# chunhualiao/Smith-Waterman

Hardware: AMD Instinct MI355X
Metric: GCUPS (DP cell updates/s) on NxN random DNA pair (higher is better)
Workload: dtype int32; 1 GPU; 16384x16384 random DNA pair (reference generator, seed 1+rank), linear gap 3/-3/-2, int32 H + int32 P written to HBM, arg-max tracked; per_gpu=one pair per GPU, max_pos=268369846, max_score=11583, grid=256, column_tiles=1, strips=131, placement_held_gib=0, preheat_fills=640

## Files before the change

smith-waterman_amd/csrc/sw_debug.h:

```cpp
#pragma once

namespace swk {

enum DebugFlag : int {
    DBG_NO_STORES = 1 << 0,
    DBG_PRODUCER_ONLY = 1 << 1,
    DBG_GENERIC_PRODUCER = 1 << 2,
    DBG_SKIP_STRIP1 = 1 << 3,
    DBG_NO_PERM = 1 << 4,
    DBG_NO_POLL_BACKOFF = 1 << 5,
    DBG_WAVE_PLACEMENT = 1 << 6,
    DBG_BLOCK_STAMPS = 1 << 7,
    DBG_NO_CONSUMER_LOOP = 1 << 8,
    DBG_EDGE_DUMP = 1 << 9,
    DBG_EPOCH8_WRAP_EARLY = 1 << 10,
    DBG_POISON_HALO = 1 << 11,
    DBG_ONE_IMPORTER = 1 << 12,
    DBG_PROGRESS_FORM = 1 << 13,
    DBG_NO_TWO_COLUMNS = 1 << 14,
    DBG_FORCE_TWO_COLUMNS = 1 << 15,
    DBG_BATCH_SINGLE_PAIR = 1 << 16,
    DBG_NO_SCOUTS = 1 << 17,
    DBG_BATCH_NO_WAVE16 = 1 << 18,
    DBG_NO_TILES = 1 << 19,
    DBG_NO_SPLIT = 1 << 20,
    DBG_BATCH_NO_PACKED_P = 1 << 21,
    DBG_S2_SCOUTS_NO_EXPORT = 1 << 21,
    DBG_S2_SYNTH_HALO = 1 << 22,
    DBG_NO_XCD_DEALING = 1 << 23,
    DBG_S2_IMPORTERS = 3 << 24,
    DBG_NO_PACING = 1 << 27,
    DBG_S2_BARRIER_SCAN = 1 << 28,
    DBG_S2_SCAN_ALL = 1 << 29,
};
constexpr int DBG_S2_IMPORTERS_SHIFT = 24;
constexpr int DBG_BATCH_MASK = DBG_NO_STORES | DBG_PRODUCER_ONLY | DBG_GENERIC_PRODUCER;

}
```

smith-waterman_amd/csrc/sw_systolic2.inc:

```

constexpr int S2_W = 126;
template <bool OV> __device__ __forceinline__ constexpr int s2_stride() { return OV ? 110 : S2_W; }
template <bool OV> __device__ __forceinline__ constexpr int s2_xlane() { return s2_stride<OV>() >> 1; }

struct S2Side {
    __attribute__((aligned(16))) u32 halo[SY_RH];
    __attribute__((aligned(16))) u32 lowv[128];
    int topv[128];
    int prod_u, halo_ready, never, pad;
};
struct Sys2Lds {
    __attribute__((aligned(16))) unsigned char ringA[64 * SY_LSTR];
    __attribute__((aligned(16))) unsigned char ringB[64 * SY_LSTR];
    __attribute__((aligned(16))) int cons_blk[8];
    S2Side side;
};

#define P2_STEP(GA, GB, GA1, GB1, TAP, TAN, TBP, TBN, HIN, SA, SB, BYTE)                                                   \
    "v_add_u32 v121, v121, %[ngap]\n\t"                                                                                   \
    "v_max3_i32 v120, " TBP ", " GB1 ", v121\n\t"                                                                         \
    "v_max3_i32 v122, " TAP ", " GB1 ", v121\n\t"                                                                         \
    "v_add_u32_sdwa " TBN ", " GB1 ", sext(" SA ") dst_sel:DWORD dst_unused:UNUSED_PAD src0_sel:DWORD src1_sel:" BYTE "\n\t" \
    "v_max_i32_dpp " GA ", v120, " GA1 " wave_shr:1 row_mask:0xf bank_mask:0xf\n\t"                                       \
    "v_max3_i32 " GB ", v122, " GA ", " HIN "\n\t"                                                                        \
// ... 109 lines not shown
    "s_cbranch_scc1 LgoB" #KB "_%=\n\t"                                                                                   \
    "s_add_i32 s89, s89, 1\n\t"                                                                                           \
    "s_add_i32 s95, s95, 1\n\t"                                                                                           \
    "s_cmp_lt_u32 s89, 0x1000000\n\t"                                                                                     \
    "s_cbranch_scc1 LpollB" #KB "_%=\n\t"                                                                                 \
    "s_branch Lfail_%=\n"

#define C2_P32(PA, PB, PP, POL) "buffer_store_dwordx2 " PP ", %[voffP], %[rP], s82 offen" POL "\n\t"
#define C2_P8(PA, PB, PP, POL)                                                                                             \
    "buffer_store_byte " PA ", %[voffP], %[rP], s82 offen" POL "\n\t"                                                      \
    "buffer_store_byte " PB ", %[voffP], %[rP], s82 offen offset:1" POL "\n\t"
#define C2_NOTRK(HA, HB, K2) ""
#define C2_TRK(HA, HB, K2)                                                                                                 \
    "v_cmp_gt_i32_e64 s[72:73], " HA ", %[bv]\n\t"                                                                         \
    "v_max_i32 %[bv], %[bv], " HA "\n\t"                                                                                   \
    "v_cndmask_b32_e64 %[bi], %[bi], " K2 ", s[72:73]\n\t"                                                                 \
    "v_cmp_gt_i32_e64 s[72:73], " HB ", %[bv]\n\t"                                                                         \
    "v_max_i32 %[bv], %[bv], " HB "\n\t"                                                                                   \
    "v_cndmask_b32_e64 %[bi], %[bi], " K2 "+1, s[72:73]\n\t"
#define C2_ROW(GA0, GA1, GB0, GB1, CH, BYTE, HA, HB, HP, PA, PB, PP, POL, HST, PST, TRK, K2)                                    \
    "v_sub_u32 %[nz], %[nz], %[ngap]\n\t"                                                                                 \
    "v_cmp_eq_u32_sdwa s[68:69], %[aA], " CH " src0_sel:DWORD src1_sel:" BYTE "\n\t"                                       \
    "v_cmp_eq_u32_sdwa s[70:71], %[aB], " CH " src0_sel:DWORD src1_sel:" BYTE "\n\t"                                       \
    "v_add_u32 " HA ", " GA1 ", %[nz]\n\t"                                                                                \
    "v_add3_u32 " HB ", " GB1 ", %[nz], v112\n\t"                                                                     \
    "v_cndmask_b32_e64 v113, %[xm], %[mm], s[68:69]\n\t"                                                                  \
    "v_cndmask_b32_e64 v114, %[xm], %[mm], s[70:71]\n\t"                                                                  \
    HST(HP, POL)                                                                                                           \
    "v_cmp_eq_u32_e64 s[60:61], " GA0 ", " GA1 "\n\t"                                                                     \
    "v_cmp_eq_u32_e64 s[64:65], " GB0 ", " GB1 "\n\t"                                                                     \
    "v_add_u32_dpp v115, " GB0 ", v113 wave_shr:1 row_mask:0xf bank_mask:0xf bound_ctrl:0\n\t"                            \
    "v_add_u32 v116, " GA0 ", v114\n\t"                                                                                   \
    "v_cndmask_b32_e64 " PA ", 2, 1, s[60:61]\n\t"                                                                        \
    "v_cndmask_b32_e64 " PB ", 2, 1, s[64:65]\n\t"                                                                        \
    "v_cmp_eq_u32_e64 s[62:63], v115, " GA1 "\n\t"                                                                        \
    "v_cmp_eq_u32_e64 s[66:67], v116, " GB1 "\n\t"                                                                        \
    "v_max3_i32 %[bm], %[bm], " HA ", " HB "\n\t"                                                                         \
    "v_cmp_eq_u32_e64 s[68:69], 0, " HA "\n\t"                                                                            \
    "v_cndmask_b32_e64 " PA ", " PA ", 3, s[62:63]\n\t"                                                                   \
    "v_cndmask_b32_e64 " PB ", " PB ", 3, s[66:67]\n\t"                                                                   \
    "v_cmp_eq_u32_e64 s[70:71], 0, " HB "\n\t"                                                                            \
    "s_add_u32 s80, s80, %[rowbH]\n\t"                                                                                    \
    "v_cndmask_b32_e64 " PA ", " PA ", 0, s[68:69]\n\t"                                                                   \
    TRK(HA, HB, K2)                                                                                                        \
    "v_cndmask_b32_e64 " PB ", " PB ", 0, s[70:71]\n\t"                                                                   \
    PST(PA, PB, PP, POL)                                                                                                   \
    "s_add_u32 s82, s82, %[rowbP]\n\t"
#define C2_H32(HP, POL) "buffer_store_dwordx2 " HP ", %[voffH], %[rH], s80 offen" POL "\n\t"
#define C2_H64(HP, POL) "buffer_store_dwordx4 " HP ", %[voffH], %[rH], s80 offen" POL "\n\t"
#define C2_EV32(GA0, GA1, GB0, GB1, CH, BYTE, POL, PST, TRK, K2) C2_ROW(GA0, GA1, GB0, GB1, CH, BYTE, "v100", "v101", "v[100:101]", "v102", "v103", "v[102:103]", POL, C2_H32, PST, TRK, K2)
#define C2_OD32(GA0, GA1, GB0, GB1, CH, BYTE, POL, PST, TRK, K2) C2_ROW(GA0, GA1, GB0, GB1, CH, BYTE, "v104", "v105", "v[104:105]", "v106", "v107", "v[106:107]", POL, C2_H32, PST, TRK, K2)
#define C2_EV64(GA0, GA1, GB0, GB1, CH, BYTE, POL, PST, TRK, K2) C2_ROW(GA0, GA1, GB0, GB1, CH, BYTE, "v100", "v102", "v[100:103]", "v104", "v105", "v[104:105]", POL, C2_H64, PST, TRK, K2)
#define C2_OD64(GA0, GA1, GB0, GB1, CH, BYTE, POL, PST, TRK, K2) C2_ROW(GA0, GA1, GB0, GB1, CH, BYTE, "v106", "v108", "v[106:109]", "v110", "v111", "v[110:111]", POL, C2_H64, PST, TRK, K2)
#define C2_RD(K, KB, OFF) "ds_read_b32 v" #K ", %[ea] offset:" #OFF "\n\tds_read_b32 v" #KB ", %[eb] offset:" #OFF "\n\t"
#define C2_RDW(K, KB, I)                                                                                                   \
    "v_add_u32 v98, " #I ", %[ew]\n\t"                                                                                   \
    "v_and_b32 v98, 1020, v98\n\t"                                                                                        \
    "v_add_u32 v99, v98, %[eb]\n\t"                                                                                       \
    "v_add_u32 v98, v98, %[ea]\n\t"                                                                                       \
    "ds_read_b32 v" #K ", v98\n\t"                                                                                        \
    "ds_read_b32 v" #KB ", v99\n\t"
#define C2_READS_FLAT                                                                                                      \
    C2_RD(64, 81, 0) C2_RD(65, 82, 4) C2_RD(66, 83, 8) C2_RD(67, 84, 12) C2_RD(68, 85, 16) C2_RD(69, 86, 20) C2_RD(70, 87, 24) C2_RD(71, 88, 28)      \
    C2_RD(72, 89, 32) C2_RD(73, 90, 36) C2_RD(74, 91, 40) C2_RD(75, 92, 44) C2_RD(76, 93, 48) C2_RD(77, 94, 52) C2_RD(78, 95, 56) C2_RD(79, 96, 60) \
    C2_RD(80, 97, 64)
#define C2_READS_WRAP                                                                                                      \
    C2_RDW(64, 81, 0) C2_RDW(65, 82, 4) C2_RDW(66, 83, 8) C2_RDW(67, 84, 12) C2_RDW(68, 85, 16) C2_RDW(69, 86, 20) C2_RDW(70, 87, 24)              \
    C2_RDW(71, 88, 28) C2_RDW(72, 89, 32) C2_RDW(73, 90, 36) C2_RDW(74, 91, 40) C2_RDW(75, 92, 44) C2_RDW(76, 93, 48) C2_RDW(77, 94, 52)            \
    C2_RDW(78, 95, 56) C2_RDW(79, 96, 60) C2_RDW(80, 97, 64)
#define C2_ASM(READS, POL, PST, TRK, C2_EV, C2_OD)                                                                                       \
    asm volatile(                                                                                                          \
        "s_load_dwordx4 s[76:79], %[cptr], 0x0\n\t"                                                                       \
        READS                                                                                                              \
        "ds_write_b32 %[slot], %[qv]\n\t"            \
        "s_mov_b32 s80, 0\n\t"                                                                                            \
        "s_mov_b32 s82, 0\n\t"                                                                                            \
        "v_sub_u32 v112, 0, %[ngap]\n\t"                                                                                  \
        "v_mov_b32 v101, 0\n\tv_mov_b32 v103, 0\n\tv_mov_b32 v107, 0\n\tv_mov_b32 v109, 0\n\t"    \
        "s_waitcnt lgkmcnt(0)\n\t"                                    \
        "s_cmp_lg_u32 %[first], 0\n\t"                                                                                    \
        "s_cbranch_scc0 Lc2_%=\n\t"                                                                                       \
        "v_mov_b32 v64, %[g0a]\n\t"                  \
        "v_mov_b32 v81, %[g0b]\n"                                                                                          \
        "Lc2_%=:\n\t"                                                                                                     \
        C2_EV("v64", "v65", "v81", "v82", "s76", "BYTE_0", POL, PST, TRK, "0") C2_OD("v65", "v66", "v82", "v83", "s76", "BYTE_1", POL, PST, TRK, "2")       \
        C2_EV("v66", "v67", "v83", "v84", "s76", "BYTE_2", POL, PST, TRK, "4") C2_OD("v67", "v68", "v84", "v85", "s76", "BYTE_3", POL, PST, TRK, "6")       \
        C2_EV("v68", "v69", "v85", "v86", "s77", "BYTE_0", POL, PST, TRK, "8") C2_OD("v69", "v70", "v86", "v87", "s77", "BYTE_1", POL, PST, TRK, "10")      \
        C2_EV("v70", "v71", "v87", "v88", "s77", "BYTE_2", POL, PST, TRK, "12") C2_OD("v71", "v72", "v88", "v89", "s77", "BYTE_3", POL, PST, TRK, "14")     \
        C2_EV("v72", "v73", "v89", "v90", "s78", "BYTE_0", POL, PST, TRK, "16") C2_OD("v73", "v74", "v90", "v91", "s78", "BYTE_1", POL, PST, TRK, "18")     \
        C2_EV("v74", "v75", "v91", "v92", "s78", "BYTE_2", POL, PST, TRK, "20") C2_OD("v75", "v76", "v92", "v93", "s78", "BYTE_3", POL, PST, TRK, "22")     \
        C2_EV("v76", "v77", "v93", "v94", "s79", "BYTE_0", POL, PST, TRK, "24") C2_OD("v77", "v78", "v94", "v95", "s79", "BYTE_1", POL, PST, TRK, "26")     \
        C2_EV("v78", "v79", "v95", "v96", "s79", "BYTE_2", POL, PST, TRK, "28") C2_OD("v79", "v80", "v96", "v97", "s79", "BYTE_3", POL, PST, TRK, "30")     \
        "v_mov_b32 %[gla], v80\n\t"                      \
        "v_mov_b32 %[glb], v97\n\t"                                                                                       \
        : [nz] "+v"(nz), [bm] "+v"(bm), [bv] "+v"(bv), [bi] "+v"(bi), [gla] "=&v"(gla), [glb] "=&v"(glb)                    \
        : [ea] "v"(ea), [eb] "v"(eb), [ew] "v"(ew), [slot] "v"(slot_addr), [qv] "v"(qv), [first] "s"(first), [g0a] "v"(g0a), [g0b] "v"(g0b),  \
          [aA] "v"(aA), [aB] "v"(aB), [mm] "v"(mm_v), [xm] "v"(xm_v), [ngap] "v"(ngap_v), [voffH] "v"(voffH),           \
          [voffP] "v"(voffP), [rH] "s"(rH), [rP] "s"(rP), [rowbH] "s"(rowbH), [rowbP] "s"(rowbP), [cptr] "s"(chars)           \
        : "vcc", "scc", "memory", "s60", "s61", "s62", "s63", "s64", "s65", "s66", "s67", "s68", "s69", "s70", "s71", "s72", "s73", "s76", "s77", "s78", "s79", \
          "s80", "s82", "v64", "v65", "v66", "v67", "v68", "v69", "v70", "v71", "v72", "v73", "v74", "v75", "v76", "v77", "v78", "v79", "v80", "v81", "v82",    \
          "v83", "v84", "v85", "v86", "v87", "v88", "v89", "v90", "v91", "v92", "v93", "v94", "v95", "v96", "v97", "v98", "v99", "v100", "v101", "v102", \
          "v103", "v104", "v105", "v106", "v107", "v108", "v109", "v110", "v111", "v112", "v113", "v114", "v115", "v116")
struct C2Out { u32 bm, gla, glb; };
__device__ __forceinline__ C2Out consumer_block2(bool flat, bool nt, bool p8, bool trk, bool h64, u32 ea, u32 eb, u32 ew, u32 slot_addr, u32 qv, int first, u32 g0a,
                                                 u32 g0b, u32& nz, u32& bv, u32& bi, u32 aA, u32 aB, u32 mm_v, u32 xm_v, u32 ngap_v, u32 voffH,
                                                 u32 voffP, sw_i32x4 rH, sw_i32x4 rP, u32 rowbH, u32 rowbP, const unsigned char* chars) {
    u32 bm = 0, gla, glb;
#define C2_PICK(READS)                                                                                                     \
    if (h64) {                                                           \
        if (p8) { if (nt) { C2_ASM(READS, " nt", C2_P8, C2_NOTRK, C2_EV64, C2_OD64); } else { C2_ASM(READS, "", C2_P8, C2_NOTRK, C2_EV64, C2_OD64); } }        \
        else { if (nt) { C2_ASM(READS, " nt", C2_P32, C2_NOTRK, C2_EV64, C2_OD64); } else { C2_ASM(READS, "", C2_P32, C2_NOTRK, C2_EV64, C2_OD64); } }         \
    } else if (trk) {                                                                                                      \
        if (p8) { if (nt) { C2_ASM(READS, " nt", C2_P8, C2_TRK, C2_EV32, C2_OD32); } else { C2_ASM(READS, "", C2_P8, C2_TRK, C2_EV32, C2_OD32); } }            \
        else { if (nt) { C2_ASM(READS, " nt", C2_P32, C2_TRK, C2_EV32, C2_OD32); } else { C2_ASM(READS, "", C2_P32, C2_TRK, C2_EV32, C2_OD32); } }             \
    } else {                                                                                                               \
        if (p8) { if (nt) { C2_ASM(READS, " nt", C2_P8, C2_NOTRK, C2_EV32, C2_OD32); } else { C2_ASM(READS, "", C2_P8, C2_NOTRK, C2_EV32, C2_OD32); } }        \
        else { if (nt) { C2_ASM(READS, " nt", C2_P32, C2_NOTRK, C2_EV32, C2_OD32); } else { C2_ASM(READS, "", C2_P32, C2_NOTRK, C2_EV32, C2_OD32); } }         \
    }
    if (flat) { C2_PICK(C2_READS_FLAT) } else { C2_PICK(C2_READS_WRAP) }
#undef C2_PICK
    return C2Out{bm, gla, glb};
}

#include "sw_wholeline_consumer.inc"

#include "sw_filler_producer.inc"


#define P2S_TAIL(GB0, GB3, H0, H3, WO, HADDR)                                                                              \
    "buffer_store_dwordx4 v[" GB0 ":" GB3 "], v97, s[76:79], s75 offen offset:" WO P2S_EXP_MOD "\n\t"                       \
    "ds_read_b128 v[" H0 ":" H3 "], " HADDR "\n\t"
#define P2S_LGKM "3"
#ifndef P2S_VMCNT
// ... 58 lines not shown
                const uint64_t now = __builtin_amdgcn_s_memrealtime();
                if (t0 == 0) t0 = now;
                if (((now - t0) >> 10) > (uint64_t)p.top_wait_ticks)
                    __hip_atomic_store((gu32*)p.abort_flag, 1u, __ATOMIC_RELAXED, __HIP_MEMORY_SCOPE_AGENT);
                if (__builtin_amdgcn_readfirstlane((int)__hip_atomic_load((gu32*)p.abort_flag, __ATOMIC_RELAXED, __HIP_MEMORY_SCOPE_AGENT)) != 0) break;
            }
        }
        tv = (int)(u32)gr;
    } else if (p.top && want) {
        tv = p.top[jt];
    }
    sd.topv[tid] = tv;
}

struct S2Pace {
    bool on = false, set = false;
    int S = 0, s = 0, steps = 0, bps = 0;
    float inv = 0.f, start = 0.f;
    __device__ __forceinline__ void calibrate(const FillParams& p, float t_first) {
        int tau_ps = p.filler_tau_ps, hop_ps = p.filler_hop_ps, bw_gbs = p.filler_bw_gbs;
        asm volatile("" : "+s"(tau_ps), "+s"(hop_ps), "+s"(bw_gbs));
        const float tau_min = (float)tau_ps * 1e-4f, hop_host = (float)hop_ps * 1e-4f;
        const float bw_per_tick = (float)bw_gbs * 10.f, fsteps = (float)steps;
        const float hop = (s >= 8) ? fminf(fmaxf(t_first / (float)s, 0.5f * hop_host), 1.5f * hop_host) : hop_host;
        start = (s >= 8) ? t_first : (float)s * hop;
        const float esteps = p.filler_end_steps > 0 ? (float)p.filler_end_steps : fsteps;
        const float wsteps = p.filler_full_steps > 0 ? (float)p.filler_full_steps : fsteps;
        const float d_chain = (float)(S - 1) * hop + esteps * tau_min;
        const float x = bw_per_tick * hop / ((float)max(bps, 1) * wsteps);
        const float d_bw = (x < 20.f) ? (float)S * hop / (1.f - __expf(-x)) : 0.f;
        const float d = fmaxf(d_chain, d_bw);
        inv = (d > start + 1.f) ? fsteps / (d - start) : 0.f;
        set = true;
    }
};
template <bool OV>
__device__ __forceinline__ bool s2_importer(S2Side& sd, const FillParams& p, int s_real, int phi, int UT, int rows, int gb, int ngap, int lane, bool synth = false,
                                            S2Pace pace = S2Pace(), int stop_u = 0x7fffffff) {
    const int s = synth ? 0 : s_real;
    __builtin_amdgcn_s_setprio(2);
    const u32 row0v = (u32)(gb + sd.topv[0] + ngap * s_real * s2_stride<OV>());
    const int xl = s2_xlane<OV>();
    const int ulast = min(UT + 64, stop_u);
    const u32 tag = (u32)gb >> 24;
    const u32* e4 = (s > 0) ? p.edge4 + (int64_t)(s - 1) * p.e4stride : nullptr;
    int impu = 1;
    bool wide = true;
    Spin spin; spin.code = 3;
    const uint64_t pace_t0 = __builtin_amdgcn_s_memrealtime();
    while (impu <= ulast) {
        const int front = lds_load(&sd.halo_ready);
        if (front > 1) impu = max(impu, front);
        if (impu > ulast) break;
        int lim = min(ulast + 1, lds_load(&sd.prod_u) + SY_RH / 2 - 2 * SY_U);
        if (pace.set && pace.inv > 0.f) lim = min(lim, 64 + max(0, (int)(((float)(uint32_t)(__builtin_amdgcn_s_memrealtime() - pace_t0) - pace.start) * pace.inv)));
        int base = impu;
        auto windows = [&](auto NB) {
            constexpr int nbat = decltype(NB)::value;
            u32 vals[nbat];
            bool oks[nbat];
#pragma unroll
            for (int b4 = 0; b4 < nbat; ++b4) {
                const int u = impu + b4 * 64 + lane;
                const int r = u - phi;
                u32 v = row0v;
                bool ok = true;
                if (r > rows) v = (u32)gb;
                else if (r > 0) {
                    if (s == 0) v = (u32)(gb + ngap * r + (p.tile_left ? p.tile_left[(int64_t)r * p.M] : 0));
                    else {
                        v = __hip_atomic_load((gu32*)(e4 + u + xl), __ATOMIC_RELAXED, __HIP_MEMORY_SCOPE_AGENT);
                        ok = (v >> 24) == tag;
                    }
                }
                vals[b4] = v;
                oks[b4] = ok && (u < lim);
            }
            const int front2 = lds_load(&sd.halo_ready);
#pragma unroll
            for (int b4 = 0; b4 < nbat; ++b4) {
                const int u = impu + b4 * 64 + lane;
                const u64 okm = __ballot(oks[b4]);
                const int npre = (okm == ~0ull) ? 64 : __builtin_ctzll(~okm);
                if (base == impu + b4 * 64 && npre > 0) {
                    if (lane < npre && (front2 <= 1 || u >= front2)) {
                        __hip_atomic_store(&sd.halo[(u - 1) & (SY_RH - 1)], vals[b4], __ATOMIC_RELAXED, __HIP_MEMORY_SCOPE_WORKGROUP);
                        __hip_atomic_store(&sd.halo[(u - 1 + SY_RH / 2) & (SY_RH - 1)], 0u, __ATOMIC_RELAXED, __HIP_MEMORY_SCOPE_WORKGROUP);
                    }
                    base += npre;
                }
            }
        };
        if (wide) windows(std::integral_constant<int, 4>{});
        else windows(std::integral_constant<int, 1>{});
        wide = (base - impu) >= 64;
        if (base > impu) {
            asm volatile("" ::: "memory");
            if (pace.on && !pace.set && base > phi + 1)
                pace.calibrate(p, (float)(uint32_t)(__builtin_amdgcn_s_memrealtime() - pace_t0));
            impu = base;
            __hip_atomic_fetch_max(&sd.halo_ready, impu, __ATOMIC_RELAXED, __HIP_MEMORY_SCOPE_WORKGROUP);
        } else if (spin.fail(p.abort_flag)) {
            return false;
        }
    }
    __builtin_amdgcn_s_setprio(0);
    return true;
}
// ... 471 lines not shown
                const bool nostore = (p.debug_flags & DBG_NO_STORES) != 0;
                const bool nt = p.store_nt != 0, store_h = H != nullptr && !nostore, store_p = P != nullptr && !nostore, trk = H == nullptr;
                const u32 voffH = (okB && store_h) ? (u32)jA * (h64 ? 8u : 4u) : SY_OOB, voffP = (okB && store_p) ? (u32)jA * (p8 ? 1u : 4u) : SY_OOB;
                const u32 rowbH = (u32)(M * (h64 ? 8 : 4)), rowbP = (u32)(M * (p8 ? 1 : 4));
                int bestcode = 0;
                constexpr int W = s2_stride<OV>();
                const bool allod = (M & 1) == 0;
                const bool wlaunch = OV && H != nullptr && !(P != nullptr && p8 && (h64 || allod)) && !trk && !p.bot_gran && !has_top &&
                                     ((uintptr_t)H & (h64 ? 15u : 7u)) == 0 && ((uintptr_t)P & 7u) == 0;
                const bool wl = wlaunch && s > 0 && s < S - 1;
                const bool mine = !OV || wlaunch || s == S - 1 || lane <= (W >> 1);
                u32 wm = 0;
                if (wl) {
                    const int64_t c1 = (int64_t)s * W + 1;
                    const u32 f0H = (u32)(((uint64_t)(uintptr_t)H + (uint64_t)(((M + c1) * 4) << hsh)) & 63u), f0P = (u32)(((uint64_t)(uintptr_t)P + (uint64_t)((M + c1) * 4)) & 63u);
                    const u32 pszH = h64 ? 16u : 8u, spanH = h64 ? 880u : 440u;
#pragma nounroll
                    for (int k = 0; k < SY_U; ++k) {
                        const bool odr = allod || (k & 1);
                        const u32 pcH = pszH * (u32)(lane - 1) - (odr ? pszH / 2 : 0u), pcP = 8u * (u32)(lane - 1) - (odr ? 4u : 0u);
                        if (!((u32)(pcH - ((f0H + (u32)k * rowbH + pcH) & 63u)) < spanH)) wm |= 1u << k;
                        if (!((u32)(pcP - ((f0P + (u32)k * rowbP + pcP) & 63u)) < 440u)) wm |= 1u << (16 + k);
                    }
                }
                if (has_top && store_h && k9 == 0) {
                    if (h64) {
                        if (okA) ((int64_t*)H)[jA] = topA;
                        if (okB) ((int64_t*)H)[jB] = topB;
                        if (s == 0 && lane == 0) ((int64_t*)H)[0] = topB;
                    } else {
                        if (okA) H[jA] = topA;
                        if (okB) H[jB] = topB;
                        if (s == 0 && lane == 0) H[0] = topB;
                    }
                }
                for (int q = q_lo + k9; q < nblk; q += nc_eff) {
                    const int qs = __builtin_amdgcn_readfirstlane(q);
                    const int r0 = qs * SY_U + 1;
                    const int need = r0 + SY_U - 1 + 63 + phi;
                    if (sf && q == q_lo + k9 && need > 256) {
                        if (!s2_importer<OV>(sd, p, s, phi, UT, rows, gb, ngap, lane, false, S2Pace(), need - 192)) return;
                    }
                    while (lds_load(&sd.prod_u) < need)
                        if (spin.fail(p.abort_flag)) return;
                    asm volatile("" ::: "memory");
                    const u32 e0 = (u32)(r0 - 2 + lane + phi);
                    const bool flat = (((u32)(r0 - 2 + phi) & (SY_R - 1)) + 63 + SY_U) < (u32)SY_R;
                    const uint64_t bH = (uint64_t)(uintptr_t)(H + (((int64_t)r0 * M) << hsh)), bP = (uint64_t)(uintptr_t)(P + (int64_t)r0 * M * (p8 ? 1 : 4));
                    const int nbr = min(SY_U, rows - r0 + 1);
                    const int nrH = nbr == SY_U ? 0x7FFFFF00 : nbr * (int)rowbH, nrP = nbr == SY_U ? 0x7FFFFF00 : nbr * (int)rowbP;
                    const sw_i32x4 dH = {__builtin_amdgcn_readfirstlane((int)(u32)bH), __builtin_amdgcn_readfirstlane((int)(u32)(bH >> 32)), nrH, 0x00020000};
                    const sw_i32x4 dP = {__builtin_amdgcn_readfirstlane((int)(u32)bP), __builtin_amdgcn_readfirstlane((int)(u32)(bP >> 32)), nrP, 0x00020000};
                    u32 nz = (u32)(-(gb + ngap * (r0 - 1 + (int)jA)));
                    u32 bv = (u32)best, bi = 0;
                    const u32 eoff = (e0 & (SY_R - 1)) * 4u;
                    C2Out o;
                    if (wl) {
                        const int64_t c1 = (int64_t)s * W + 1;
                        const uint64_t fH = bH + (uint64_t)((c1 * 4) << hsh), fP = bP + (uint64_t)(c1 * 4);
                        const uint64_t bH2 = fH & ~(uint64_t)63, bP2 = fP & ~(uint64_t)63;
                        const u32 dlH = (u32)(bH2 - bH), dlP = (u32)(bP2 - bP);
                        const sw_i32x4 dH2 = {__builtin_amdgcn_readfirstlane((int)(u32)bH2), __builtin_amdgcn_readfirstlane((int)(u32)(bH2 >> 32)),
                                              nbr == SY_U ? 0x7FFFFF00 : __builtin_amdgcn_readfirstlane(nrH - (int)dlH), 0x00020000};
                        const sw_i32x4 dP2 = {__builtin_amdgcn_readfirstlane((int)(u32)bP2), __builtin_amdgcn_readfirstlane((int)(u32)(bP2 >> 32)),
                                              nbr == SY_U ? 0x7FFFFF00 : __builtin_amdgcn_readfirstlane(nrP - (int)dlP), 0x00020000};
                        const u32 vH = voffH == SY_OOB ? SY_OOB : voffH - dlH;
                        const u32 vP = p8 ? ((voffP == SY_OOB || lane > (W >> 1)) ? SY_OOB : voffP) : (voffP == SY_OOB ? SY_OOB : voffP - dlP);
                        o.bm = consumer_block3(flat, nt, h64, p8, flat ? laneA + eoff : laneA, flat ? laneB + eoff : laneB, eoff, slot_addr, (u32)qs,
                                               __builtin_amdgcn_readfirstlane(qs == 0 ? 1 : 0), g0a, g0b, nz, (u32)aA, (u32)aB, mm_v, xm_v, ngap_v, vH, vP,
                                               dH2, p8 ? dP : dP2, rowbH, rowbP, bchars + (r0 - 1), wm, allod);
                        o.gla = o.glb = 0u;
                    } else
                    o = consumer_block2(flat, nt, p8, trk, h64, flat ? laneA + eoff : laneA, flat ? laneB + eoff : laneB, eoff, slot_addr, (u32)qs,
                                                    __builtin_amdgcn_readfirstlane(qs == 0 ? 1 : 0), g0a, g0b, nz, bv, bi, (u32)aA, (u32)aB, mm_v, xm_v, ngap_v,
                                                    voffH, voffP, dH, dP, rowbH, rowbP, bchars + (r0 - 1));
                    if (trk) { if (okB && mine && (int)bv > best) { best = (int)bv; bestq = qs; bestcode = (int)bi; } }
                    else if (okB && mine && (int)o.bm > best) { best = (int)o.bm; bestq = qs; }
                    if (p.bot_gran && qs == nblk - 1) {
                        const int zl = gb + ngap * (rows + (int)jA);
                        if (okA) __hip_atomic_store((gu64*)(p.bot_gran + jA), ((u64)p.bot_tag << 32) | (u64)(u32)((int)o.gla - zl), __ATOMIC_RELAXED, __HIP_MEMORY_SCOPE_SYSTEM);
                        if (okB) __hip_atomic_store((gu64*)(p.bot_gran + jB), ((u64)p.bot_tag << 32) | (u64)(u32)((int)o.glb - zl - ngap), __ATOMIC_RELAXED, __HIP_MEMORY_SCOPE_SYSTEM);
                        if (s == 0 && lane == 0) __hip_atomic_store((gu64*)p.bot_gran, (u64)p.bot_tag << 32, __ATOMIC_RELAXED, __HIP_MEMORY_SCOPE_SYSTEM);
                        if (p.bot_done) {
                            __builtin_amdgcn_fence(__ATOMIC_RELEASE, "");
                            asm volatile("s_waitcnt vmcnt(0)" ::: "memory");
                            const int n63 = (int)((p.cols + 62) / 63);
                            if (lane < 2 && 2 * s + lane < n63)
                                __hip_atomic_store((gu32*)(p.bot_done + 2 * s + lane), p.bot_tag, __ATOMIC_RELAXED, __HIP_MEMORY_SCOPE_SYSTEM);
                        }
                    }
                }
                if (best > 0 && !nostore) {
                    if (trk) {
                        bestrow = bestq * SY_U + 1 + (bestcode >> 1);
                        bestcol = bestcode & 1;
                    } else {
                        __builtin_amdgcn_s_waitcnt(0);
                        const u32 psz = h64 ? 16u : 8u, span = h64 ? 880u : 440u, lc = psz * (u32)(lane - 1);
                        const u32 f0 = (u32)(((uint64_t)(uintptr_t)H + (uint64_t)(((((int64_t)bestq * SY_U + 1) * M + (int64_t)s * W + 1) * 4) << hsh)) & 63u);
                        auto inwin = [&](u32 rowoff, u32 pc) { return (u32)(pc - ((f0 + rowoff + pc) & 63u)) < span; };
                        const int nk = min(SY_U, rows - bestq * SY_U);
                        int hvA[SY_U], hvB[SY_U];
#pragma unroll
                        for (int k = 0; k < SY_U; ++k) {
                            const int64_t o = (int64_t)(bestq * SY_U + 1 + min(k, nk - 1)) * M + jA;
                            hvA[k] = (int)__builtin_nontemporal_load(&H[o << hsh]);
                            hvB[k] = (int)__builtin_nontemporal_load(&H[(o + 1) << hsh]);
                        }
#pragma unroll
                        for (int k = SY_U - 1; k >= 0; --k) {
                            bool stA = k < nk, stB = k < nk;
                            if (wl) {
                                const u32 rowoff = (u32)k * rowbH;
                                if (allod || (k & 1)) { stA = stA && inwin(rowoff, lc - psz / 2); stB = stB && lane < 63 && inwin(rowoff, lc + psz / 2); }
                                else stA = stB = stA && inwin(rowoff, lc);
                            }
                            if (stB && hvB[k] == best) { bestrow = bestq * SY_U + 1 + k; bestcol = 1; }
                            if (stA && hvA[k] == best) { bestrow = bestq * SY_U + 1 + k; bestcol = 0; }
                        }
                        if (bestrow == 0 && wlaunch) best = 0;
                    }
                }
            } else
            for (int q = q_lo + k9; q < nblk; q += nc_eff) {
                const int r0 = q * SY_U + 1;
                const int need = r0 + SY_U - 1 + 63 + phi;
                while (lds_load(&sd.prod_u) < need)
// ... 106 lines not shown
```

smith-waterman_amd/csrc/sw_wholeline_consumer.inc:

```

#define C3_MASK(BIT, VOFF)                                                                                                 \
    "v_bfe_i32 v124, %[wm], " BIT ", 1\n\t"                                                                                \
    "v_or_b32 v120, v124, " VOFF "\n\t"
#define C3_ROW(GA0, GA1, GB0, GB1, CH, BYTE, HA, HB, PA, PB, HST, PST)                                                     \
    "v_sub_u32 %[nz], %[nz], %[ngap]\n\t"                                                                                 \
    "v_cmp_eq_u32_sdwa s[68:69], %[aA], " CH " src0_sel:DWORD src1_sel:" BYTE "\n\t"                                       \
    "v_cmp_eq_u32_sdwa s[70:71], %[aB], " CH " src0_sel:DWORD src1_sel:" BYTE "\n\t"                                       \
    "v_add_u32 " HA ", " GA1 ", %[nz]\n\t"                                                                                \
    "v_add3_u32 " HB ", " GB1 ", %[nz], v112\n\t"                                                                         \
    "v_cndmask_b32_e64 v113, %[xm], %[mm], s[68:69]\n\t"                                                                  \
    "v_cndmask_b32_e64 v114, %[xm], %[mm], s[70:71]\n\t"                                                                  \
    HST                                                                                                                    \
    "v_cmp_eq_u32_e64 s[60:61], " GA0 ", " GA1 "\n\t"                                                                     \
    "v_cmp_eq_u32_e64 s[64:65], " GB0 ", " GB1 "\n\t"                                                                     \
    "v_add_u32_dpp v115, " GB0 ", v113 wave_shr:1 row_mask:0xf bank_mask:0xf bound_ctrl:0\n\t"                            \
    "v_add_u32 v99, " GA0 ", v114\n\t"                                                                                   \
    "v_cndmask_b32_e64 " PA ", 2, 1, s[60:61]\n\t"                                                                        \
    "v_cndmask_b32_e64 " PB ", 2, 1, s[64:65]\n\t"                                                                        \
    "v_cmp_eq_u32_e64 s[62:63], v115, " GA1 "\n\t"                                                                        \
    "v_cmp_eq_u32_e64 s[66:67], v99, " GB1 "\n\t"                                                                        \
    "v_max3_i32 %[bm], %[bm], " HA ", " HB "\n\t"                                                                         \
    "v_cmp_eq_u32_e64 s[68:69], 0, " HA "\n\t"                                                                            \
    "v_cndmask_b32_e64 " PA ", " PA ", 3, s[62:63]\n\t"                                                                   \
    "v_cndmask_b32_e64 " PB ", " PB ", 3, s[66:67]\n\t"                                                                   \
    "v_cmp_eq_u32_e64 s[70:71], 0, " HB "\n\t"                                                                            \
    "s_add_u32 s80, s80, %[rowbH]\n\t"                                                                                    \
    "v_cndmask_b32_e64 " PA ", " PA ", 0, s[68:69]\n\t"                                                                   \
    "v_cndmask_b32_e64 " PB ", " PB ", 0, s[70:71]\n\t"                                                                   \
    PST                                                                                                                    \
    "s_add_u32 s82, s82, %[rowbP]\n\t"
#define C3_EV32(GA0, GA1, GB0, GB1, CH, BYTE, POL, KH, KP)                                                                         \
    C3_ROW(GA0, GA1, GB0, GB1, CH, BYTE, "v100", "v101", "v102", "v103",                                                   \
           C3_MASK(KH, "%[voffH]") "buffer_store_dwordx2 v[100:101], v120, %[rH], s80 offen" POL "\n\t",  \
           C3_MASK(KP, "%[voffP]") "buffer_store_dwordx2 v[102:103], v120, %[rP], s82 offen" POL "\n\t")
#define C3_EV32P8(GA0, GA1, GB0, GB1, CH, BYTE, POL, KH, KP)                                                                       \
    C3_ROW(GA0, GA1, GB0, GB1, CH, BYTE, "v100", "v101", "v102", "v103",                                                   \
           C3_MASK(KH, "%[voffH]") "buffer_store_dwordx2 v[100:101], v120, %[rH], s80 offen" POL "\n\t",                    \
           "buffer_store_byte v102, %[voffP], %[rP], s82 offen\n\tbuffer_store_byte v103, %[voffP], %[rP], s82 offen offset:1\n\t")
#define C3_OD32P8(GA0, GA1, GB0, GB1, CH, BYTE, POL, KH, KP)                                                                       \
    C3_ROW(GA0, GA1, GB0, GB1, CH, BYTE, "v119", "v121", "v123", "v125",                                                   \
           "v_mov_b32_dpp v118, v121 wave_shr:1 row_mask:0xf bank_mask:0xf bound_ctrl:0\n\t"                              \
           C3_MASK(KH, "v116") "buffer_store_dwordx2 v[118:119], v120, %[rH], s80 offen" POL "\n\t",                        \
           "buffer_store_byte v123, %[voffP], %[rP], s82 offen\n\tbuffer_store_byte v125, %[voffP], %[rP], s82 offen offset:1\n\t")
#define C3_EV64(GA0, GA1, GB0, GB1, CH, BYTE, POL, KH, KP)                                                                         \
    C3_ROW(GA0, GA1, GB0, GB1, CH, BYTE, "v100", "v102", "v104", "v105",                                                   \
           C3_MASK(KH, "%[voffH]") "buffer_store_dwordx4 v[100:103], v120, %[rH], s80 offen" POL "\n\t",  \
           C3_MASK(KP, "%[voffP]") "buffer_store_dwordx2 v[104:105], v120, %[rP], s82 offen" POL "\n\t")
#define C3_OD_P(POL, KP)                                                                                                       \
           C3_MASK(KP, "v117")    \
           "v_mov_b32_dpp v122, v125 wave_shr:1 row_mask:0xf bank_mask:0xf bound_ctrl:0\n\t"                              \
           "buffer_store_dwordx2 v[122:123], v120, %[rP], s82 offen" POL "\n\t"
#define C3_OD32(GA0, GA1, GB0, GB1, CH, BYTE, POL, KH, KP)                                                                         \
    C3_ROW(GA0, GA1, GB0, GB1, CH, BYTE, "v119", "v121", "v123", "v125",                                                   \
           "v_mov_b32_dpp v118, v121 wave_shr:1 row_mask:0xf bank_mask:0xf bound_ctrl:0\n\t"                              \
           C3_MASK(KH, "v116") "buffer_store_dwordx2 v[118:119], v120, %[rH], s80 offen" POL "\n\t", \
           C3_OD_P(POL, KP))
#define C3_OD64(GA0, GA1, GB0, GB1, CH, BYTE, POL, KH, KP)                                                                         \
    C3_ROW(GA0, GA1, GB0, GB1, CH, BYTE, "v108", "v110", "v123", "v125",                                                   \
           "v_mov_b32_dpp v106, v110 wave_shr:1 row_mask:0xf bank_mask:0xf bound_ctrl:0\n\t"                              \
           C3_MASK(KH, "v116") "buffer_store_dwordx4 v[106:109], v120, %[rH], s80 offen" POL "\n\t", \
           C3_OD_P(POL, KP))
#define C3_ASM(READS, POL, C3_EV, C3_OD, HALFH)                                                                                   \
    asm volatile(                                                                                                          \
        "s_load_dwordx4 s[76:79], %[cptr], 0x0\n\t"                                                                       \
        READS                                                                                                              \
        "ds_write_b32 %[slot], %[qv]\n\t"            \
        "s_mov_b32 s80, 0\n\t"                                                                                            \
        "s_mov_b32 s82, 0\n\t"                                                                                            \
        "v_sub_u32 v112, 0, %[ngap]\n\t"                                                                                  \
        "v_add_u32 v116, " HALFH ", %[voffH]\n\t"                  \
        "v_add_u32 v117, -4, %[voffP]\n\t"                                                                                \
        "v_mov_b32 v101, 0\n\tv_mov_b32 v103, 0\n\tv_mov_b32 v107, 0\n\tv_mov_b32 v109, 0\n\tv_mov_b32 v111, 0\n\t"    \
        "s_waitcnt lgkmcnt(0)\n\t"                                    \
        "s_cmp_lg_u32 %[first], 0\n\t"                                                                                    \
        "s_cbranch_scc0 Lc3_%=\n\t"                                                                                       \
        "v_mov_b32 v64, %[g0a]\n\t"                  \
        "v_mov_b32 v81, %[g0b]\n"                                                                                          \
        "Lc3_%=:\n\t"                                                                                                     \
        C3_EV("v64", "v65", "v81", "v82", "s76", "BYTE_0", POL, "0", "16") C3_OD("v65", "v66", "v82", "v83", "s76", "BYTE_1", POL, "1", "17")     \
        C3_EV("v66", "v67", "v83", "v84", "s76", "BYTE_2", POL, "2", "18") C3_OD("v67", "v68", "v84", "v85", "s76", "BYTE_3", POL, "3", "19")     \
        C3_EV("v68", "v69", "v85", "v86", "s77", "BYTE_0", POL, "4", "20") C3_OD("v69", "v70", "v86", "v87", "s77", "BYTE_1", POL, "5", "21")     \
        C3_EV("v70", "v71", "v87", "v88", "s77", "BYTE_2", POL, "6", "22") C3_OD("v71", "v72", "v88", "v89", "s77", "BYTE_3", POL, "7", "23")     \
        C3_EV("v72", "v73", "v89", "v90", "s78", "BYTE_0", POL, "8", "24") C3_OD("v73", "v74", "v90", "v91", "s78", "BYTE_1", POL, "9", "25")     \
        C3_EV("v74", "v75", "v91", "v92", "s78", "BYTE_2", POL, "10", "26") C3_OD("v75", "v76", "v92", "v93", "s78", "BYTE_3", POL, "11", "27")     \
        C3_EV("v76", "v77", "v93", "v94", "s79", "BYTE_0", POL, "12", "28") C3_OD("v77", "v78", "v94", "v95", "s79", "BYTE_1", POL, "13", "29")     \
        C3_EV("v78", "v79", "v95", "v96", "s79", "BYTE_2", POL, "14", "30") C3_OD("v79", "v80", "v96", "v97", "s79", "BYTE_3", POL, "15", "31")     \
        : [nz] "+v"(nz), [bm] "+v"(bm)                                                                                      \
        : [ea] "v"(ea), [eb] "v"(eb), [ew] "v"(ew), [slot] "v"(slot_addr), [qv] "v"(qv), [first] "s"(first), [g0a] "v"(g0a), [g0b] "v"(g0b),  \
          [aA] "v"(aA), [aB] "v"(aB), [mm] "v"(mm_v), [xm] "v"(xm_v), [ngap] "v"(ngap_v), [voffH] "v"(voffH),           \
          [voffP] "v"(voffP), [wm] "v"(wm), [rH] "s"(rH), [rP] "s"(rP), [rowbH] "s"(rowbH), [rowbP] "s"(rowbP), [cptr] "s"(chars)     \
        : "vcc", "scc", "memory", "s60", "s61", "s62", "s63", "s64", "s65", "s66", "s67", "s68", "s69", "s70", "s71", "s72", "s73", "s76", "s77", "s78", "s79", \
          "s80", "s82",                                \
          "v64", "v65", "v66", "v67", "v68", "v69", "v70", "v71", "v72", "v73", "v74", "v75", "v76", "v77", "v78", "v79", "v80", "v81", "v82",    \
          "v83", "v84", "v85", "v86", "v87", "v88", "v89", "v90", "v91", "v92", "v93", "v94", "v95", "v96", "v97", "v98", "v99", "v100", "v101", "v102", \
          "v103", "v104", "v105", "v106", "v107", "v108", "v109", "v110", "v111", "v112", "v113", "v114", "v115", "v116", "v117", "v118", "v119", "v120", \
          "v121", "v122", "v123", "v124", "v125", "v126", "v127")
__device__ __forceinline__ u32 consumer_block3(bool flat, bool nt, bool h64, bool p8, u32 ea, u32 eb, u32 ew, u32 slot_addr, u32 qv, int first, u32 g0a, u32 g0b, u32& nz,
                                               u32 aA, u32 aB, u32 mm_v, u32 xm_v, u32 ngap_v, u32 voffH, u32 voffP, sw_i32x4 rH, sw_i32x4 rP,
                                               u32 rowbH, u32 rowbP, const unsigned char* chars, u32 wm, bool allod) {
    u32 bm = 0;
#define C3_PICK(READS)                                                                                                     \
    if (p8) {                                                                       \
        if (nt) { C3_ASM(READS, " nt", C3_EV32P8, C3_OD32P8, "-4"); } else { C3_ASM(READS, "", C3_EV32P8, C3_OD32P8, "-4"); }           \
    } else if (allod) {                                                                                                    \
        if (h64) { if (nt) { C3_ASM(READS, " nt", C3_OD64, C3_OD64, "-8"); } else { C3_ASM(READS, "", C3_OD64, C3_OD64, "-8"); } }    \
        else { if (nt) { C3_ASM(READS, " nt", C3_OD32, C3_OD32, "-4"); } else { C3_ASM(READS, "", C3_OD32, C3_OD32, "-4"); } }        \
    } else if (h64) { if (nt) { C3_ASM(READS, " nt", C3_EV64, C3_OD64, "-8"); } else { C3_ASM(READS, "", C3_EV64, C3_OD64, "-8"); } } \
    else { if (nt) { C3_ASM(READS, " nt", C3_EV32, C3_OD32, "-4"); } else { C3_ASM(READS, "", C3_EV32, C3_OD32, "-4"); } }
    if (flat) { C3_PICK(C2_READS_FLAT) } else { C3_PICK(C2_READS_WRAP) }
#undef C3_PICK
    return bm;
}
```

Baseline: 337.9 GCUPS.

## Pair LDS ring reads with ds_read2 and sleep importers when blocked

Replaces the 34 single ds_read_b32 loads in the flat consumer ring read with paired ds_read2_b32 instructions, halving the LDS instruction count. Importer waves that cannot advance, because they are blocked by the ring limit or by pacing, now drop priority and s_sleep for a duration scaled to the pacing rate instead of spinning, which frees issue slots for compute waves. A debug bit that skips ring reads is also added, routed through the first flag. The sleeps may add latency when the producer advances sooner than expected.

```diff
diff --git a/smith-waterman_amd/csrc/sw_debug.h b/smith-waterman_amd/csrc/sw_debug.h
--- a/smith-waterman_amd/csrc/sw_debug.h
+++ b/smith-waterman_amd/csrc/sw_debug.h
@@ -29,9 +29,11 @@
     DBG_S2_SYNTH_HALO = 1 << 22,
     DBG_NO_XCD_DEALING = 1 << 23,
     DBG_S2_IMPORTERS = 3 << 24,
+    DBG_S2_NO_RING_READS = 1 << 26,
     DBG_NO_PACING = 1 << 27,
     DBG_S2_BARRIER_SCAN = 1 << 28,
     DBG_S2_SCAN_ALL = 1 << 29,
+    DBG_S2_IMPORTERS_POLL = 1 << 30,
 };
 constexpr int DBG_S2_IMPORTERS_SHIFT = 24;
 constexpr int DBG_BATCH_MASK = DBG_NO_STORES | DBG_PRODUCER_ONLY | DBG_GENERIC_PRODUCER;
diff --git a/smith-waterman_amd/csrc/sw_systolic2.inc b/smith-waterman_amd/csrc/sw_systolic2.inc
--- a/smith-waterman_amd/csrc/sw_systolic2.inc
+++ b/smith-waterman_amd/csrc/sw_systolic2.inc
@@ -185,7 +185,7 @@
 #define C2_OD32(GA0, GA1, GB0, GB1, CH, BYTE, POL, PST, TRK, K2) C2_ROW(GA0, GA1, GB0, GB1, CH, BYTE, "v104", "v105", "v[104:105]", "v106", "v107", "v[106:107]", POL, C2_H32, PST, TRK, K2)
 #define C2_EV64(GA0, GA1, GB0, GB1, CH, BYTE, POL, PST, TRK, K2) C2_ROW(GA0, GA1, GB0, GB1, CH, BYTE, "v100", "v102", "v[100:103]", "v104", "v105", "v[104:105]", POL, C2_H64, PST, TRK, K2)
 #define C2_OD64(GA0, GA1, GB0, GB1, CH, BYTE, POL, PST, TRK, K2) C2_ROW(GA0, GA1, GB0, GB1, CH, BYTE, "v106", "v108", "v[106:109]", "v110", "v111", "v[110:111]", POL, C2_H64, PST, TRK, K2)
-#define C2_RD(K, KB, OFF) "ds_read_b32 v" #K ", %[ea] offset:" #OFF "\n\tds_read_b32 v" #KB ", %[eb] offset:" #OFF "\n\t"
+#define C2_RD2(K0, K1, ADDR, O0, O1) "ds_read2_b32 v[" #K0 ":" #K1 "], %[" #ADDR "] offset0:" #O0 " offset1:" #O1 "\n\t"
 #define C2_RDW(K, KB, I)                                                                                                   \
     "v_add_u32 v98, " #I ", %[ew]\n\t"                                                                                   \
     "v_and_b32 v98, 1020, v98\n\t"                                                                                        \
@@ -194,9 +194,12 @@
     "ds_read_b32 v" #K ", v98\n\t"                                                                                        \
     "ds_read_b32 v" #KB ", v99\n\t"
 #define C2_READS_FLAT                                                                                                      \
-    C2_RD(64, 81, 0) C2_RD(65, 82, 4) C2_RD(66, 83, 8) C2_RD(67, 84, 12) C2_RD(68, 85, 16) C2_RD(69, 86, 20) C2_RD(70, 87, 24) C2_RD(71, 88, 28)      \
-    C2_RD(72, 89, 32) C2_RD(73, 90, 36) C2_RD(74, 91, 40) C2_RD(75, 92, 44) C2_RD(76, 93, 48) C2_RD(77, 94, 52) C2_RD(78, 95, 56) C2_RD(79, 96, 60) \
-    C2_RD(80, 97, 64)
+    "ds_read_b32 v81, %[eb]\n\t"                                                                                         \
+    C2_RD2(64, 65, ea, 0, 1) C2_RD2(82, 83, eb, 1, 2) C2_RD2(66, 67, ea, 2, 3) C2_RD2(84, 85, eb, 3, 4)                    \
+    C2_RD2(68, 69, ea, 4, 5) C2_RD2(86, 87, eb, 5, 6) C2_RD2(70, 71, ea, 6, 7) C2_RD2(88, 89, eb, 7, 8)                    \
+    C2_RD2(72, 73, ea, 8, 9) C2_RD2(90, 91, eb, 9, 10) C2_RD2(74, 75, ea, 10, 11) C2_RD2(92, 93, eb, 11, 12)               \
+    C2_RD2(76, 77, ea, 12, 13) C2_RD2(94, 95, eb, 13, 14) C2_RD2(78, 79, ea, 14, 15) C2_RD2(96, 97, eb, 15, 16)            \
+    "ds_read_b32 v80, %[ea] offset:64\n\t"
 #define C2_READS_WRAP                                                                                                      \
     C2_RDW(64, 81, 0) C2_RDW(65, 82, 4) C2_RDW(66, 83, 8) C2_RDW(67, 84, 12) C2_RDW(68, 85, 16) C2_RDW(69, 86, 20) C2_RDW(70, 87, 24)              \
     C2_RDW(71, 88, 28) C2_RDW(72, 89, 32) C2_RDW(73, 90, 36) C2_RDW(74, 91, 40) C2_RDW(75, 92, 44) C2_RDW(76, 93, 48) C2_RDW(77, 94, 52)            \
@@ -204,14 +207,17 @@
 #define C2_ASM(READS, POL, PST, TRK, C2_EV, C2_OD)                                                                                       \
     asm volatile(                                                                                                          \
         "s_load_dwordx4 s[76:79], %[cptr], 0x0\n\t"                                                                       \
+        "s_bitcmp1_b32 %[first], 1\n\t"              \
+        "s_cbranch_scc1 Lnr_%=\n\t"                                                                                       \
         READS                                                                                                              \
+        "Lnr_%=:\n\t"                                                                                                     \
         "ds_write_b32 %[slot], %[qv]\n\t"            \
         "s_mov_b32 s80, 0\n\t"                                                                                            \
         "s_mov_b32 s82, 0\n\t"                                                                                            \
         "v_sub_u32 v112, 0, %[ngap]\n\t"                                                                                  \
         "v_mov_b32 v101, 0\n\tv_mov_b32 v103, 0\n\tv_mov_b32 v107, 0\n\tv_mov_b32 v109, 0\n\t"    \
         "s_waitcnt lgkmcnt(0)\n\t"                                    \
-        "s_cmp_lg_u32 %[first], 0\n\t"                                                                                    \
+        "s_bitcmp1_b32 %[first], 0\n\t"                                               \
         "s_cbranch_scc0 Lc2_%=\n\t"                                                                                       \
         "v_mov_b32 v64, %[g0a]\n\t"                  \
         "v_mov_b32 v81, %[g0b]\n"                                                                                          \
@@ -376,8 +382,23 @@
         const int front = lds_load(&sd.halo_ready);
         if (front > 1) impu = max(impu, front);
         if (impu > ulast) break;
-        int lim = min(ulast + 1, lds_load(&sd.prod_u) + SY_RH / 2 - 2 * SY_U);
+        const int ring_lim = lds_load(&sd.prod_u) + SY_RH / 2 - 2 * SY_U;
+        int lim = min(ulast + 1, ring_lim);
         if (pace.set && pace.inv > 0.f) lim = min(lim, 64 + max(0, (int)(((float)(uint32_t)(__builtin_amdgcn_s_memrealtime() - pace_t0) - pace.start) * pace.inv)));
+        if (impu >= lim && !(p.debug_flags & DBG_S2_IMPORTERS_POLL)) {
+            __builtin_amdgcn_s_setprio(0);
+            if (lim == ring_lim) __builtin_amdgcn_s_sleep(60);
+            else {
+                if (pace.inv <= 0.125f) __builtin_amdgcn_s_sleep(48);
+                else if (pace.inv <= 0.25f) __builtin_amdgcn_s_sleep(24);
+                else if (pace.inv <= 0.5f) __builtin_amdgcn_s_sleep(12);
+                else __builtin_amdgcn_s_sleep(6);
+            }
+            wide = false;
+            if (spin.fail(p.abort_flag)) return false;
+            __builtin_amdgcn_s_setprio(2);
+            continue;
+        }
         int base = impu;
         auto windows = [&](auto NB) {
             constexpr int nbat = decltype(NB)::value;
@@ -955,6 +976,9 @@
                     const sw_i32x4 dH = {__builtin_amdgcn_readfirstlane((int)(u32)bH), __builtin_amdgcn_readfirstlane((int)(u32)(bH >> 32)), nrH, 0x00020000};
                     const sw_i32x4 dP = {__builtin_amdgcn_readfirstlane((int)(u32)bP), __builtin_amdgcn_readfirstlane((int)(u32)(bP >> 32)), nrP, 0x00020000};
                     u32 nz = (u32)(-(gb + ngap * (r0 - 1 + (int)jA)));
+                    int noread = p.debug_flags;
+                    asm volatile("" : "+s"(noread));
+                    noread = (noread >> 25) & 2;
                     u32 bv = (u32)best, bi = 0;
                     const u32 eoff = (e0 & (SY_R - 1)) * 4u;
                     C2Out o;
@@ -970,12 +994,12 @@
                         const u32 vH = voffH == SY_OOB ? SY_OOB : voffH - dlH;
                         const u32 vP = p8 ? ((voffP == SY_OOB || lane > (W >> 1)) ? SY_OOB : voffP) : (voffP == SY_OOB ? SY_OOB : voffP - dlP);
                         o.bm = consumer_block3(flat, nt, h64, p8, flat ? laneA + eoff : laneA, flat ? laneB + eoff : laneB, eoff, slot_addr, (u32)qs,
-                                               __builtin_amdgcn_readfirstlane(qs == 0 ? 1 : 0), g0a, g0b, nz, (u32)aA, (u32)aB, mm_v, xm_v, ngap_v, vH, vP,
+                                               __builtin_amdgcn_readfirstlane((qs == 0 ? 1 : 0) | noread), g0a, g0b, nz, (u32)aA, (u32)aB, mm_v, xm_v, ngap_v, vH, vP,
                                                dH2, p8 ? dP : dP2, rowbH, rowbP, bchars + (r0 - 1), wm, allod);
                         o.gla = o.glb = 0u;
                     } else
                     o = consumer_block2(flat, nt, p8, trk, h64, flat ? laneA + eoff : laneA, flat ? laneB + eoff : laneB, eoff, slot_addr, (u32)qs,
-                                                    __builtin_amdgcn_readfirstlane(qs == 0 ? 1 : 0), g0a, g0b, nz, bv, bi, (u32)aA, (u32)aB, mm_v, xm_v, ngap_v,
+                                                    __builtin_amdgcn_readfirstlane((qs == 0 ? 1 : 0) | noread), g0a, g0b, nz, bv, bi, (u32)aA, (u32)aB, mm_v, xm_v, ngap_v,
                                                     voffH, voffP, dH, dP, rowbH, rowbP, bchars + (r0 - 1));
                     if (trk) { if (okB && mine && (int)bv > best) { best = (int)bv; bestq = qs; bestcode = (int)bi; } }
                     else if (okB && mine && (int)o.bm > best) { best = (int)o.bm; bestq = qs; }
diff --git a/smith-waterman_amd/csrc/sw_wholeline_consumer.inc b/smith-waterman_amd/csrc/sw_wholeline_consumer.inc
--- a/smith-waterman_amd/csrc/sw_wholeline_consumer.inc
+++ b/smith-waterman_amd/csrc/sw_wholeline_consumer.inc
@@ -63,7 +63,10 @@
 #define C3_ASM(READS, POL, C3_EV, C3_OD, HALFH)                                                                                   \
     asm volatile(                                                                                                          \
         "s_load_dwordx4 s[76:79], %[cptr], 0x0\n\t"                                                                       \
+        "s_bitcmp1_b32 %[first], 1\n\t"              \
+        "s_cbranch_scc1 Lnr_%=\n\t"                                                                                       \
         READS                                                                                                              \
+        "Lnr_%=:\n\t"                                                                                                     \
         "ds_write_b32 %[slot], %[qv]\n\t"            \
         "s_mov_b32 s80, 0\n\t"                                                                                            \
         "s_mov_b32 s82, 0\n\t"                                                                                            \
@@ -72,7 +75,7 @@
         "v_add_u32 v117, -4, %[voffP]\n\t"                                                                                \
         "v_mov_b32 v101, 0\n\tv_mov_b32 v103, 0\n\tv_mov_b32 v107, 0\n\tv_mov_b32 v109, 0\n\tv_mov_b32 v111, 0\n\t"    \
         "s_waitcnt lgkmcnt(0)\n\t"                                    \
-        "s_cmp_lg_u32 %[first], 0\n\t"                                                                                    \
+        "s_bitcmp1_b32 %[first], 0\n\t"                                               \
         "s_cbranch_scc0 Lc3_%=\n\t"                                                                                       \
         "v_mov_b32 v64, %[g0a]\n\t"                  \
         "v_mov_b32 v81, %[g0b]\n"                                                                                          \
```

Result: no change. 337.5 GCUPS (-0.1%).
